# 236088/reflect-sampling-nerf

Measured on AMD Instinct MI355X. Metric: rays/sec (train step) at 4096 rays x 128 samples, 1/2/4/8 MI355X; PSNR vs ref, higher is better.
Workload: dtype f32

## Files before the change

### reflect_sampling_nerf_amd/csrc/rsn_field_bwd.hip

```cpp
#include "rsn_mfma.h"

#include "rsn_field_common.h"
#include "rsn_field_bwd_common.h"

template <int NB, int MMA>
__global__ __launch_bounds__(256) void rsn_field_bwd_kernel(const BwdJobs J) {
  constexpr bool FOLD = MMA == RSN_MMA_F32_FOLDED;
  constexpr int MODE = FOLD ? 0 : MMA;
  constexpr int HIT = FOLD ? 16 : NB * 4;
  constexpr int XITS = (NB * 4 > 16) ? NB * 4 : 16;
  constexpr int WAVE_F4 = (XITS + RSN_AUX_ITS) * 64;
  constexpr int W = NB * 32;
  constexpr bool SBF = MODE == 3;
  __shared__ float4 smem[4 * WAVE_F4];

  const int lane = threadIdx.x & 63;
  const int wid = __builtin_amdgcn_readfirstlane(threadIdx.x >> 6);
  float4* X = smem + wid * WAVE_F4 + lane;
  float* Xf = reinterpret_cast<float*>(X);

  const BwdShared& P = J.s;
  const TileJobs T = tile_space<128>(J);
  const float* __restrict__ pk = P.packed;
  const float4 zero4 = make_float4(0.0f, 0.0f, 0.0f, 0.0f);

  for (long long gtile = blockIdx.x; gtile < T.n_tiles; gtile += gridDim.x) {
    const TileAt ta = tile_at(T, gtile);
    const BwdJob& a = J.j[ta.job];
    const long long n_points = ta.n_points, tile = ta.tile;
    const long long p0 = tile * 128 + wid * 32;
    if (p0 >= n_points) continue;
    int ln = lane;
    asm volatile("" : "+v"(ln));
    const int m = ln & 31, h = ln >> 5;
    const long long p = p0 + m;
    const bool valid = p < n_points;
    const long long pc = valid ? p : n_points - 1;
    const int rows = (int)(n_points - p0 < 32 ? n_points - p0 : 32);
    constexpr bool LOOPST = MODE == 0;
    auto rb_epi = [&](float* base, long long elem, int row_elems) {
      return rowbuf<SBF>(LOOPST ? nullptr : base, elem, rows, row_elems, m, h);
    };
    auto rb_loop = [&](float* base, long long elem, int row_elems) {
      return rowbuf<false>(LOOPST ? base : nullptr, elem, rows, row_elems, m, h);
    };
    const float live = valid ? 1.0f : 0.0f;

    auto bits_at = [&](int l) -> const unsigned* {
      return a.saved.relu_bits + ((((long long)l * (a.act_stride / W)) + pc) * 2 + h) * (NB / 2 > 2 ? NB / 2 : 2);
    };
    HeadGradIn hg;
    head_grad_inputs(a, pc, live, h == 1 && valid, hg);

    X[0] = (h == 1) ? make_float4(hg.dz[0], hg.dz[1], hg.dz[2], 0.0f) : zero4;
    X[64] = zero4; X[128] = zero4; X[192] = zero4;
    {
      const ReluBits<4> mb = load_relu_bits<4>(bits_at(P.num_layers));
      __builtin_amdgcn_sched_barrier(0);
      f32x16 acc[4];
      zero_acc<4>(acc);
      gemm_mode<MODE, 4, 4, true>(acc, pk + P.L.wT_rgb, pk + P.L.hT_rgb, X, 4, ln);
      store_masked_bits<4, SBF>(acc, X, mb, h, rb_epi(a.gout.da_mid, p0 * 128, 128));
    }
    if constexpr (!FOLD) {
      f32x16 acc[NB];
      zero_acc<NB>(acc);
      gemm_mode<MODE, NB, NB, true>(acc, pk + P.L.wT_mid_x, pk + P.L.hT_mid_x, X, 16, ln, rb_loop(a.gout.da_mid, p0 * 128, 128));
      store_act<NB, NB, false, SBF>(acc, X, rb_epi(a.gout.d_bott, p0 * W, W), h);
    }
    {
      const float4 q0 = head_grad_row<false>(h == 0 ? 0 : 1, a, P.density_bias, pc, live, hg);
      const float4 q1 = head_grad_row<false>(h == 0 ? 2 : 3, a, P.density_bias, pc, live, hg);
      X[(HIT + 0) * 64] = q0;
      X[(HIT + 1) * 64] = q1;
      X[(HIT + 2) * 64] = zero4;
      X[(HIT + 3) * 64] = zero4;
      if (valid && a.gout.dz_heads) {
        *reinterpret_cast<float4*>(a.gout.dz_heads + pc * 16 + 4 * h) = q0;
        *reinterpret_cast<float4*>(a.gout.dz_heads + pc * 16 + 8 + 4 * h) = q1;
      }
      const int l = P.num_layers - 1;
      const ReluBits<NB> mb = load_relu_bits<NB>(bits_at(l));
      __builtin_amdgcn_sched_barrier(0);
      f32x16 acc[NB];
      zero_acc<NB>(acc);
      if constexpr (FOLD)
        gemm_mode<MODE, NB, NB, true>(acc, pk + P.L.wT_fold, pk + P.L.hT_bh, X, 16 + 4, ln, rb_loop(a.gout.da_mid, p0 * 128, 128));
      else
        gemm_mode<MODE, NB, NB, true>(acc, pk + P.L.wT_bh, pk + P.L.hT_bh, X, NB * 4 + 4, ln, rb_loop(a.gout.d_bott, p0 * W, W));
      store_masked_bits<NB, SBF>(acc, X, mb, h, rb_epi(a.gout.dy, (long long)l * a.act_stride + p0 * W, W));
    }
    f32x16 eacc[4];
    zero_acc<4>(eacc);
#pragma unroll 1
    for (int l = P.num_layers - 1; l >= 1; --l) {
      if (a.need_input_grad && l == P.skip_layer)
        gemm_mode<MODE, 4, 4, true>(eacc, pk + P.L.wT_enc_skip, pk + P.L.hT_enc_skip, X, NB * 4, ln);
      const ReluBits<NB> mb = load_relu_bits<NB>(bits_at(l - 1));
      __builtin_amdgcn_sched_barrier(0);
      f32x16 acc[NB];
      zero_acc<NB>(acc);
      gemm_mode<MODE, NB, NB, true>(acc, pk + P.L.wT_x[l], pk + P.L.hT_x[l], X, NB * 4, ln,
                          rb_loop(a.gout.dy, (long long)l * a.act_stride + p0 * W, W));
      store_masked_bits<NB, SBF>(acc, X, mb, h, rb_epi(a.gout.dy, (long long)(l - 1) * a.act_stride + p0 * W, W));
    }
    if (LOOPST && !a.need_input_grad) {
      const RowBuf r0 = rb_loop(a.gout.dy, p0 * W, W);
#pragma unroll 4
      for (int it = 0; it < NB * 4; ++it) sv_put_it(r0, it, X[it * 64]);
    }
    if (a.need_input_grad) {
      gemm_mode<MODE, 4, 4, true>(eacc, pk + P.L.wT_enc0, pk + P.L.hT_enc0, X, NB * 4, ln, rb_loop(a.gout.dy, p0 * W, W));
      store_act<4, 4, false>(eacc, X);
      const float* encp = a.saved.enc + pc * RSN_K_ENC_PAD;
      float dvar[3];
#pragma unroll 1
      for (int c = 0; c < 3; ++c) {
        float part = 0.0f;
#pragma unroll 2
        for (int jj = 0; jj < 8; ++jj) {
          const float f = h ? P.freqs[8 + jj] : P.freqs[jj];
          const int u = c * 8 + jj, u2 = u + 24;
          const float gs = Xf[(u >> 2) * 256 + (u & 3)], gc = Xf[(u2 >> 2) * 256 + (u2 & 3)];
          const float fs = encp[(u >> 2) * 8 + 4 * h + (u & 3)], fc = encp[(u2 >> 2) * 8 + 4 * h + (u2 & 3)];
          part += (-0.5f * (f * f)) * (gs * fs + gc * fc);
        }
        const float tot = part + __shfl_xor(part, 32, 64);
        if (c == 0) dvar[0] = tot; else if (c == 1) dvar[1] = tot; else dvar[2] = tot;
      }
      if (h == 0 && valid && a.gout.d_input) a.gout.d_input[pc] = input_grad_of_dvar(a, pc, dvar);
    }
  }
}

static int launch_bwd_jobs(const rsn_field_desc* d, const float* packed, BwdJob* js, int n, void* stream) {
  RSN_REQUIRE(n >= 1 && n <= RSN_MAX_JOBS, RSN_ERR_INVALID_ARGUMENT, "n_jobs=%d (1..%d)", n, RSN_MAX_JOBS);
  BwdJobs J = {};
  RSN_TRY(rsn_fill_shared(J.s, d, packed));
  for (int k = 0; k < n; ++k) {
    BwdJob& a = js[k];
    RSN_REQUIRE(a.saved.relu_bits && a.saved.heads && a.gout.dy, RSN_ERR_INVALID_ARGUMENT,
                "job %d: saved relu_bits / heads and gout.dy are required", k);
    RSN_REQUIRE(!a.need_input_grad || (a.saved.enc && a.gout.d_input), RSN_ERR_INVALID_ARGUMENT,
                "job %d: need_input_grad needs saved.enc and gout.d_input", k);
    RSN_REQUIRE(a.mode == RSN_MODE_INF || (a.fwd.raw_density && a.fwd.diff && a.fwd.tint), RSN_ERR_INVALID_ARGUMENT,
// ... 94 lines not shown
```

### reflect_sampling_nerf_amd/csrc/rsn_mfma.h

```cpp
#pragma once
#include "rsn_common.h"

typedef float f32x16 __attribute__((ext_vector_type(16)));

#define RSN_MODE_FRUSTUM 0
#define RSN_MODE_INF 1
#define RSN_MODE_GAUSS 2
#define RSN_MODE_EMB 3

__device__ __forceinline__ float softplus_f(float x) { return x > 20.0f ? x : log1pf(expf(x)); }
__device__ __forceinline__ float sigmoid_f(float x) { return 1.0f / (1.0f + expf(-x)); }

__device__ __forceinline__ float sincos_big(float a, int quad) {
  const float q = rintf(a * 0.63661977236758134308f);
  float r = __builtin_fmaf(-q, 1.5707963705062866f, a);
  r = __builtin_fmaf(-q, -4.371138828673793e-08f, r);
  r = __builtin_fmaf(-q, -1.7151245100058819e-15f, r);
  const int n = (int)q + quad;
  const float s = r * r;
  const float ps = r + r * s * (-1.6666654611e-1f + s * (8.3321608736e-3f + s * (-1.9515295891e-4f)));
  const float pc =
      1.0f + s * (-0.5f + s * (4.166664568298827e-2f + s * (-1.388731625493765e-3f + s * 2.443315711809948e-5f)));
  const float v = (n & 1) ? pc : ps;
  return (n & 2) ? -v : v;
// ... 176 lines not shown
  int it = 0;
#pragma unroll 1
  for (; it + 2 < n_it; it += 3) {
    load_w<NBO, NBT>(wc, wp, cl(it + 2));
    b1 = xl[cl(it + 1) * 64];
    mma4<NBO>(acc, wa, b0);
    if (sv_on(save)) sv_put_it(save, it, b0);
    interleave_loads<NBO>();
    __builtin_amdgcn_sched_barrier(0);
    load_w<NBO, NBT>(wa, wp, cl(it + 3));
    b2 = xl[cl(it + 2) * 64];
    mma4<NBO>(acc, wb, b1);
    if (sv_on(save)) sv_put_it(save, it + 1, b1);
    interleave_loads<NBO>();
    __builtin_amdgcn_sched_barrier(0);
    load_w<NBO, NBT>(wb, wp, cl(it + 4));
    b0 = xl[cl(it + 3) * 64];
    mma4<NBO>(acc, wc, b2);
    if (sv_on(save)) sv_put_it(save, it + 2, b2);
    interleave_loads<NBO>();
    __builtin_amdgcn_sched_barrier(0);
  }
  if (it < n_it) {
    mma4<NBO>(acc, wa, b0);
    if (sv_on(save)) sv_put_it(save, it, b0);
  }
  if (it + 1 < n_it) {
    b1 = xl[(it + 1) * 64];
    mma4<NBO>(acc, wb, b1);
    if (sv_on(save)) sv_put_it(save, it + 1, b1);
  }
}

template <int NBO, int NBT = NBO, class SV = const float*>
__device__ __forceinline__ void gemm_run(f32x16 (&acc)[NBO], float4 (&wa)[NBO], const float* __restrict__ wseg,
                                          const float4* xl, int n_it, int lane, SV save = nullptr) {
  const WBuf wp = wbuf_make(wseg, lane);
  float4 wb[NBO];
  float4 ba, bb;
  ba = xl[0];
  int it = 0;
#pragma unroll 1
  for (; it + 1 < n_it; it += 2) {
    load_w<NBO, NBT>(wb, wp, it + 1);
    bb = xl[(it + 1) * 64];
    mma4<NBO>(acc, wa, ba);
    if (sv_on(save)) sv_put_it(save, it, ba);
    interleave_loads<NBO>();
    __builtin_amdgcn_sched_barrier(0);
    {
      const int in = (it + 2 < n_it) ? it + 2 : n_it - 1;
      load_w<NBO, NBT>(wa, wp, in);
      ba = xl[in * 64];
    }
    mma4<NBO>(acc, wb, bb);
    if (sv_on(save)) sv_put_it(save, it + 1, bb);
    interleave_loads<NBO>();
    __builtin_amdgcn_sched_barrier(0);
  }
  if (it < n_it) {
    mma4<NBO>(acc, wa, ba);
    if (sv_on(save)) sv_put_it(save, it, ba);
  }
}

template <int NBO, int NBT = NBO, bool PF2 = false, class SV = const float*>
// ... 111 lines not shown
    xhi = xl[(2 * k2 + 1) * 64];
    __builtin_amdgcn_sched_barrier(0);
    if (H1 > 0) mma16<NBO, (H1 > 0 ? H1 : 1), (H1 > 0 ? H0 : 0), NSPLIT, FULL>(acc, wb, bc);
    __builtin_amdgcn_sched_barrier(0);
    bc = bn;
  }
}

template <int MODE, int NBO, int NBT = NBO, bool PF2 = false, class SV = const float*>
__device__ __forceinline__ void gemm_mode(f32x16 (&acc)[NBO], const float* __restrict__ w32, const float* __restrict__ w16,
                                          const float4* xl, int n_it, int lane, SV save = nullptr) {
  static_assert(MODE == 0 || NBT == NBO, "the split-bf16 loops own every output block of their segment");
  if (MODE == 0) {
    gemm<NBO, NBT, PF2>(acc, w32, xl, n_it, lane, save);
  } else {
    gemm_bf16<NBO, (MODE == 1 ? 3 : (MODE == 2 ? 2 : 1))>(acc, w16, xl, (n_it + 1) / 2, lane);
  }
}

template <int MODE, int NBO, int NBT = NBO>
__device__ __forceinline__ void pre_mode(float4 (&wa)[NBO], const float* __restrict__ w32, int lane) {
  if (MODE == 0) pre_w<NBO, NBT>(wa, w32, lane);
}

template <int MODE, int NBO, int NBT = NBO, bool PF2 = false, class SV = const float*>
__device__ __forceinline__ void gemm_mode_run(f32x16 (&acc)[NBO], float4 (&wa)[NBO], const float* __restrict__ w32,
                                              const float* __restrict__ w16, const float4* xl, int n_it, int lane,
                                              SV save = nullptr) {
  static_assert(MODE == 0 || NBT == NBO, "the split-bf16 loops own every output block of their segment");
  if (MODE == 0) {
    if (PF2) gemm_run2<NBO, NBT>(acc, wa, w32, xl, n_it, lane, save); else gemm_run<NBO, NBT>(acc, wa, w32, xl, n_it, lane, save);
  } else {
    gemm_bf16<NBO, (MODE == 1 ? 3 : (MODE == 2 ? 2 : 1))>(acc, w16, xl, (n_it + 1) / 2, lane);
  }
}

template <int NBO>
__device__ __forceinline__ void zero_acc(f32x16 (&acc)[NBO]) {
#pragma unroll
  for (int nb = 0; nb < NBO; ++nb)
#pragma unroll
    for (int r = 0; r < 16; ++r) acc[nb][r] = 0.0f;
}

__device__ __forceinline__ unsigned relu_bits16(const f32x16& a) {
  unsigned b = 0u;
#pragma unroll
  for (int r = 0; r < 16; ++r) {
    const unsigned lo = __float_as_uint(relu_f(a[r]));
    unsigned bit;
    if (r == 0) {
      asm("v_min_u32 %0, %1, 1" : "=v"(bit) : "v"(lo));
      b = bit;
    } else {
      unsigned nb;
      asm("v_min_u32 %0, %2, 1\n\tv_lshl_or_b32 %1, %0, %3, %4" : "=&v"(bit), "=v"(nb) : "v"(lo), "n"(r), "v"(b));
      b = nb;
    }
  }
  return b;
}

template <int Q>
__device__ __forceinline__ unsigned relu_bits4q(unsigned b, const float4 v) {
  const unsigned lo[4] = {__float_as_uint(v.x), __float_as_uint(v.y), __float_as_uint(v.z), __float_as_uint(v.w)};
#pragma unroll
// ... 153 lines not shown
    c = __builtin_amdgcn_mfma_f32_32x32x16_bf16(s3, b, c, 0, 0, 0);
    c = __builtin_amdgcn_mfma_f32_32x32x16_bf16(s2, b, c, 0, 0, 0);
    c = __builtin_amdgcn_mfma_f32_32x32x16_bf16(s1, b, c, 0, 0, 0);
    acc[nb0 + t] = c;
  }
}

template <int NBO>
__device__ __forceinline__ void gemm_f32_bits(f32x16 (&acc)[NBO], const float* __restrict__ w32seg, const float* __restrict__ wd,
                                              const ReluBits<NBO>& m, int lane) {
  static_assert(NBO % 2 == 0, "two fragment buffers of NBO / 2 blocks");
  constexpr int NH = NBO / 2, NK = 2 * NBO;
  const WBuf wp = wbuf_make(w32seg, lane);
  const float* __restrict__ wdl = wd + 4 * (lane >> 5);
  float4 fa[NH][2], fb[NH][2];
  load_w32_pair<NBO, NH>(fa, wp, 0, 0);
  const SeedWords mw = seed_words<NBO>(m);
  float4 dlo = *reinterpret_cast<const float4*>(wdl), dhi = *reinterpret_cast<const float4*>(wdl + 8);
#pragma unroll 1
  for (int kk = 0; kk < NK; ++kk) {
    load_w32_pair<NBO, NH>(fb, wp, kk, NH);
    const int kn = (kk + 1 < NK) ? kk + 1 : kk;
    const float4 nlo = *reinterpret_cast<const float4*>(wdl + 16 * kn), nhi = *reinterpret_cast<const float4*>(wdl + 16 * kn + 8);
    const bf16x8 bc = bits_bf16x8(mw, kk);
    mma16_bits_f32<NBO, NH>(acc, fa, dlo, dhi, bc, 0);
    __builtin_amdgcn_sched_barrier(0);
    load_w32_pair<NBO, NH>(fa, wp, kn, 0);
    mma16_bits_f32<NBO, NH>(acc, fb, dlo, dhi, bc, NH);
    __builtin_amdgcn_sched_barrier(0);
    dlo = nlo; dhi = nhi;
  }
}

__device__ __forceinline__ f32x16 x9_block(f32x16 c, const BSplit& w, const BSplit& b) {
  c = __builtin_amdgcn_mfma_f32_32x32x16_bf16(w.s3, b.s3, c, 0, 0, 0);
  c = __builtin_amdgcn_mfma_f32_32x32x16_bf16(w.s3, b.s2, c, 0, 0, 0);
  c = __builtin_amdgcn_mfma_f32_32x32x16_bf16(w.s2, b.s3, c, 0, 0, 0);
  c = __builtin_amdgcn_mfma_f32_32x32x16_bf16(w.s3, b.s1, c, 0, 0, 0);
  c = __builtin_amdgcn_mfma_f32_32x32x16_bf16(w.s2, b.s2, c, 0, 0, 0);
  c = __builtin_amdgcn_mfma_f32_32x32x16_bf16(w.s1, b.s3, c, 0, 0, 0);
  c = __builtin_amdgcn_mfma_f32_32x32x16_bf16(w.s2, b.s1, c, 0, 0, 0);
  c = __builtin_amdgcn_mfma_f32_32x32x16_bf16(w.s1, b.s2, c, 0, 0, 0);
  c = __builtin_amdgcn_mfma_f32_32x32x16_bf16(w.s1, b.s1, c, 0, 0, 0);
  return c;
}

template <int NBO>
__device__ __forceinline__ void gemm_f32_x9(f32x16 (&acc)[NBO], const float* __restrict__ w32seg, const float4* xl, int n_k16,
                                            int lane) {
  static_assert(NBO % 2 == 0, "two fragment buffers of NBO / 2 blocks");
  constexpr int NH = NBO / 2;
  const WBuf wp = wbuf_make(w32seg, lane);
  float4 fa[NH][2], fb[NH][2];
  load_w32_pair<NBO, NH>(fa, wp, 0, 0);
  load_w32_pair<NBO, NH>(fb, wp, 0, NH);
  BSplit bc = split8<3>(xl[0], xl[64]);
  const int k1 = n_k16 > 1 ? 1 : 0;
  float4 xlo = xl[(2 * k1) * 64], xhi = xl[(2 * k1 + 1) * 64];
  BSplit w = split8<3>(fa[0][0], fa[0][1]);
  BSplit bn = bc;
#pragma unroll 1
  for (int kk = 0; kk < n_k16; ++kk) {
    const int kn = (kk + 1 < n_k16) ? kk + 1 : kk;
    const int k2 = (kk + 2 < n_k16) ? kk + 2 : kn;
#pragma unroll
    for (int b = 0; b < NBO; ++b) {
      BSplit wn;
      if (b + 1 < NH) wn = split8<3>(fa[b + 1][0], fa[b + 1][1]);
      else if (b + 1 < NBO) wn = split8<3>(fb[b + 1 - NH][0], fb[b + 1 - NH][1]);
      else wn = split8<3>(fa[0][0], fa[0][1]);
      if (b == NH - 1) load_w32_pair<NBO, NH>(fa, wp, kn, 0);
      if (b == NBO - 1) {
        load_w32_pair<NBO, NH>(fb, wp, kn, NH);
        bn = split8<3>(xlo, xhi);
        xlo = xl[(2 * k2) * 64];
        xhi = xl[(2 * k2 + 1) * 64];
      }
      acc[b] = x9_block(acc[b], w, bc);
      const bool loads = b == NH - 1 || b == NBO - 1;
#pragma unroll
      for (int g = 0; g < 9; ++g) {
        __builtin_amdgcn_sched_group_barrier(0x008, 1, 0);
        if (loads && g < 2 * NH) __builtin_amdgcn_sched_group_barrier(0x020, 1, 0);
        if (b == NBO - 1) __builtin_amdgcn_sched_group_barrier(0x002, 8, 0);
        else __builtin_amdgcn_sched_group_barrier(0x002, 5, 0);
      }
      if (b == NBO - 1) __builtin_amdgcn_sched_group_barrier(0x100, 2, 0);
      __builtin_amdgcn_sched_barrier(0);
      w = wn;
    }
    bc = bn;
  }
}

__device__ __forceinline__ unsigned bit_mask(int word, int pos) {
  unsigned m;
  asm("v_bfe_i32 %0, %1, %2, 1" : "=v"(m) : "v"(word), "n"(pos));
  return m;
}

template <int NBO, bool SBF = false, class SV = float*>
__device__ __forceinline__ void store_masked_bits(const f32x16 (&acc)[NBO], float4* xl, const ReluBits<NBO>& m, int h,
                                                  SV save = nullptr) {
#pragma unroll
  for (int nb = 0; nb < NBO; ++nb)
#pragma unroll
    for (int q = 0; q < 4; ++q) {
      const int word = m.w[nb / 2];
      const int base = (nb & 1) * 16 + 4 * q;
      float4 v;
      v.x = __uint_as_float(__float_as_uint(acc[nb][4 * q + 0]) & bit_mask(word, base + 0));
      v.y = __uint_as_float(__float_as_uint(acc[nb][4 * q + 1]) & bit_mask(word, base + 1));
      v.z = __uint_as_float(__float_as_uint(acc[nb][4 * q + 2]) & bit_mask(word, base + 2));
      v.w = __uint_as_float(__float_as_uint(acc[nb][4 * q + 3]) & bit_mask(word, base + 3));
      xl[(nb * 4 + q) * 64] = v;
      if (sv_on(save)) sv_put<SBF>(save, nb, q, h, v);
    }
}

template <int NBO, int NBS, bool RELU, bool SBF = false, class SV = float*>
__device__ __forceinline__ void store_act(const f32x16 (&acc)[NBO], float4* xl, SV save = nullptr, int h = 0,
                                          unsigned* bits = nullptr) {
  unsigned bw[NBS / 2 > 0 ? NBS / 2 : 1];
#pragma unroll
  for (int nb = 0; nb < NBS; ++nb) {
    unsigned b16 = 0u;
#pragma unroll
    for (int q = 0; q < 4; ++q) {
      float4 v = make_float4(acc[nb][4 * q + 0], acc[nb][4 * q + 1], acc[nb][4 * q + 2], acc[nb][4 * q + 3]);
      if (RELU) {
        v.x = relu_f(v.x);
        v.y = relu_f(v.y);
        v.z = relu_f(v.z);
        v.w = relu_f(v.w);
        b16 = relu_bits4(b16, v, q);
      }
      xl[(nb * 4 + q) * 64] = v;
      if (sv_on(save)) sv_put<SBF>(save, nb, q, h, v);
    }
    if (RELU) {
      if (nb & 1) bw[nb / 2] |= b16 << 16; else bw[nb / 2] = b16;
    }
  }
  if (RELU && bits) {
    if (NBS >= 8) {
#pragma unroll
      for (int w4 = 0; w4 < NBS / 8; ++w4)
        *reinterpret_cast<uint4*>(bits + w4 * 4) = make_uint4(bw[w4 * 4], bw[w4 * 4 + 1], bw[w4 * 4 + 2], bw[w4 * 4 + 3]);
    } else {
// ... 92 lines not shown
```

### reflect_sampling_nerf_amd/csrc/rsn_field_kernel.h

```cpp
#pragma once
#include "rsn_mfma.h"

#include "rsn_field_common.h"

template <bool X9, bool PACKED, int MODE, int NBO>
__device__ __forceinline__ void sweep_gemm(f32x16 (&acc)[NBO], const float* __restrict__ w32, const float* __restrict__ w16,
                                           const float4* xl, int n_it, int lane) {
  if constexpr (X9) {
    if constexpr (PACKED) gemm_bf16<NBO, 3, true>(acc, w16, xl, n_it / 2, lane); else gemm_f32_x9<NBO>(acc, w32, xl, n_it / 2, lane);
  } else {
    gemm_mode<MODE, NBO, NBO, true>(acc, w32, w16, xl, n_it, lane);
  }
}

template <int NB, bool TRAIN, int MMA>
__global__ __launch_bounds__(256) void rsn_field_kernel(const FieldJobs J) {
  constexpr bool FOLD = MMA == RSN_MMA_F32_FOLDED;
  constexpr int MODE = FOLD ? 0 : MMA;
  static_assert(!FOLD || TRAIN, "the folded bottleneck serves the exact-fp32 training kernels");
  constexpr int NBH = FOLD ? 5 : NB + 1;
  constexpr int XITS = (NB * 4 > 16) ? NB * 4 : 16;
  constexpr int WAVE_F4 = (XITS + RSN_AUX_ITS) * 64;
  constexpr int W = NB * 32;
  constexpr bool SBF = TRAIN && MODE == 3;
  __shared__ float4 smem[4 * WAVE_F4];

  const int lane = threadIdx.x & 63;
  const int wid = __builtin_amdgcn_readfirstlane(threadIdx.x >> 6);
  float4* X = smem + wid * WAVE_F4 + lane;
  float4* AUX = X + XITS * 64;
  float* Xf = reinterpret_cast<float*>(X);

  const FieldShared& P = J.s;
  const TileJobs T = tile_space<128>(J);
  const float* __restrict__ pk = P.packed;

  for (long long gtile = blockIdx.x; gtile < T.n_tiles; gtile += gridDim.x) {
    const TileAt ta = tile_at(T, gtile);
    const FieldJob& a = J.j[ta.job];
    const long long n_points = ta.n_points, tile = ta.tile;
    const long long p0 = tile * 128 + wid * 32;
    if (p0 >= n_points) continue;
    int ln = lane;
    asm volatile("" : "+v"(ln));
    const int m = ln & 31, h = ln >> 5;
// ... 190 lines not shown
      if (h == 1 && valid) colour_out<false, TRAIN>(a, pc, accr[0][0], accr[0][1], accr[0][2], dcol, tcol);
    }

    constexpr bool SEED_BITS = TRAIN && MODE == 0;
    if (TRAIN && a.saved.normals && a.saved.relu_bits) {
      const float* __restrict__ wd = pk + P.L.v_density;
      const bool peel = SEED_BITS && P.num_layers >= 2;
      if (peel) {
        const ReluBits<NB> m7 = load_relu_bits<NB>(bits_at(P.num_layers - 1));
        const ReluBits<NB> mb = load_relu_bits<NB>(bits_at(P.num_layers - 2));
        __builtin_amdgcn_sched_barrier(0);
        f32x16 acc[NB];
        zero_acc<NB>(acc);
        if constexpr (FOLD) {
          gemm_bf16_bits<NB>(acc, pk + P.L.hT_seed, m7, ln);
        } else {
          gemm_f32_bits<NB>(acc, pk + P.L.wT_x[P.num_layers - 1], wd, m7, ln);
        }
        store_masked_bits<NB>(acc, X, mb, h);
      } else {
        const ReluBits<NB> mb = load_relu_bits<NB>(bits_at(P.num_layers - 1));
#pragma unroll
        for (int it = 0; it < NB * 4; ++it) {
          const float4 w = *reinterpret_cast<const float4*>(wd + it * 8 + 4 * h);
          const int word = mb.w[it / 8];
          const int base = ((it / 4) & 1) * 16 + 4 * (it & 3);
          X[it * 64] = make_float4(
              __uint_as_float(__float_as_uint(w.x) & bit_mask(word, base + 0)),
              __uint_as_float(__float_as_uint(w.y) & bit_mask(word, base + 1)),
              __uint_as_float(__float_as_uint(w.z) & bit_mask(word, base + 2)),
              __uint_as_float(__float_as_uint(w.w) & bit_mask(word, base + 3)));
        }
      }
      f32x16 eacc[4];
      zero_acc<4>(eacc);
#pragma unroll 1
      for (int l = P.num_layers - (peel ? 2 : 1); l >= 1; --l) {
        if (l == P.skip_layer) sweep_gemm<SEED_BITS, FOLD, MODE, 4>(eacc, pk + P.L.wT_enc_skip, pk + P.L.hT_enc_skip, X, NB * 4, ln);
        const ReluBits<NB> mb = load_relu_bits<NB>(bits_at(l - 1));
        __builtin_amdgcn_sched_barrier(0);
        f32x16 acc[NB];
        zero_acc<NB>(acc);
        sweep_gemm<SEED_BITS, FOLD, MODE, NB>(acc, pk + P.L.wT_x[l], pk + P.L.hT_x[l], X, NB * 4, ln);
        store_masked_bits<NB>(acc, X, mb, h);
      }
      sweep_gemm<SEED_BITS, FOLD, MODE, 4>(eacc, pk + P.L.wT_enc0, pk + P.L.hT_enc0, X, NB * 4, ln);
      store_act<4, 4, false>(eacc, X);
      float nrm[3];
#pragma unroll 1
      for (int c = 0; c < 3; ++c) {
        const float x = (c == 0) ? mc[0] : (c == 1 ? mc[1] : mc[2]);
        const float v = (c == 0) ? vc[0] : (c == 1 ? vc[1] : vc[2]);
        const float sx = 6.283185307179586f * x;
        float part = 0.0f;
#pragma unroll 2
        for (int jj = 0; jj < 8; ++jj) {
          const float f = h ? P.freqs[8 + jj] : P.freqs[jj];
          const float ang = sx * f;
          const float e = has_cov ? expf(-0.5f * (v * (f * f))) : 1.0f;
          const int u = c * 8 + jj;
          const float gs = Xf[(u >> 2) * 256 + (u & 3)];
          const float gc = Xf[((u + 24) >> 2) * 256 + ((u + 24) & 3)];
          part += (gs * (e * cos_big(ang)) + gc * (e * cos_big(ang + 1.5707963267948966f))) * f;
        }
        part *= 6.283185307179586f;
        if (h == 0) part += Xf[12 * 256 + c];
        const float tot = part + __shfl_xor(part, 32, 64);
        if (c == 0) nrm[0] = tot; else if (c == 1) nrm[1] = tot; else nrm[2] = tot;
      }
      if (h == 0 && valid) {
        const float len = fmaxf(sqrtf(nrm[0] * nrm[0] + nrm[1] * nrm[1] + nrm[2] * nrm[2]), 1e-12f);
        a.saved.normals[pc * 3 + 0] = -(nrm[0] / len);
        a.saved.normals[pc * 3 + 1] = -(nrm[1] / len);
        a.saved.normals[pc * 3 + 2] = -(nrm[2] / len);
      }
    }
  }
}
```

Measured before the change: 94550.

## Chain weight prefetch across successive backward GEMM segments

Replaces each per-layer GEMM call in the backward field kernel with a chained variant. During the tail iterations of one segment it loads the first one or two weight fragments of the next segment, so every GEMM after the first starts with its weights already in registers. This targets the global-load latency bubble at each layer boundary. The cost is more live registers (fa/fb/sa/sb are kept across the tile loop) and fragile fragment bookkeeping across the FOLD, NB and need_input_grad paths, which could hurt occupancy or correctness.

```diff
diff --git a/reflect_sampling_nerf_amd/csrc/rsn_field_bwd.hip b/reflect_sampling_nerf_amd/csrc/rsn_field_bwd.hip
--- a/reflect_sampling_nerf_amd/csrc/rsn_field_bwd.hip
+++ b/reflect_sampling_nerf_amd/csrc/rsn_field_bwd.hip
@@ -23,6 +23,14 @@
   const TileJobs T = tile_space<128>(J);
   const float* __restrict__ pk = P.packed;
   const float4 zero4 = make_float4(0.0f, 0.0f, 0.0f, 0.0f);
+
+  float4 fa[NB], fb[NB], sa[4], sb[4];
+  if constexpr (MODE == 0) {
+    const WBuf wp = wbuf_make(pk + P.L.wT_rgb, lane);
+    load_w<4>(sa, wp, 0);
+    load_w<4>(sb, wp, 1);
+  }
+  constexpr const float* no_rows = nullptr;
 
   for (long long gtile = blockIdx.x; gtile < T.n_tiles; gtile += gridDim.x) {
     const TileAt ta = tile_at(T, gtile);
@@ -49,6 +57,9 @@
     auto bits_at = [&](int l) -> const unsigned* {
       return a.saved.relu_bits + ((((long long)l * (a.act_stride / W)) + pc) * 2 + h) * (NB / 2 > 2 ? NB / 2 : 2);
     };
+    auto seg_behind = [&](int l) -> const float* {
+      return pk + (l > 1 ? P.L.wT_x[l - 1] : (a.need_input_grad ? P.L.wT_enc0 : P.L.wT_rgb));
+    };
     HeadGradIn hg;
     head_grad_inputs(a, pc, live, h == 1 && valid, hg);
 
@@ -59,13 +70,15 @@
       __builtin_amdgcn_sched_barrier(0);
       f32x16 acc[4];
       zero_acc<4>(acc);
-      gemm_mode<MODE, 4, 4, true>(acc, pk + P.L.wT_rgb, pk + P.L.hT_rgb, X, 4, ln);
+      gemm_mode_chain<MODE, 4, 4, NB>(acc, sa, sb, pk + P.L.wT_rgb, pk + P.L.hT_rgb, X, ln, no_rows,
+                                      pk + (FOLD ? P.L.wT_fold : P.L.wT_mid_x), fa, fb);
       store_masked_bits<4, SBF>(acc, X, mb, h, rb_epi(a.gout.da_mid, p0 * 128, 128));
     }
     if constexpr (!FOLD) {
       f32x16 acc[NB];
       zero_acc<NB>(acc);
-      gemm_mode<MODE, NB, NB, true>(acc, pk + P.L.wT_mid_x, pk + P.L.hT_mid_x, X, 16, ln, rb_loop(a.gout.da_mid, p0 * 128, 128));
+      gemm_mode_chain<MODE, 16, NB, NB>(acc, fa, fb, pk + P.L.wT_mid_x, pk + P.L.hT_mid_x, X, ln, rb_loop(a.gout.da_mid, p0 * 128, 128),
+                                        pk + P.L.wT_bh, fa, fb);
       store_act<NB, NB, false, SBF>(acc, X, rb_epi(a.gout.d_bott, p0 * W, W), h);
     }
     {
@@ -85,9 +98,11 @@
       f32x16 acc[NB];
       zero_acc<NB>(acc);
       if constexpr (FOLD)
-        gemm_mode<MODE, NB, NB, true>(acc, pk + P.L.wT_fold, pk + P.L.hT_bh, X, 16 + 4, ln, rb_loop(a.gout.da_mid, p0 * 128, 128));
+        gemm_mode_chain<MODE, 16 + 4, NB, NB>(acc, fa, fb, pk + P.L.wT_fold, pk + P.L.hT_bh, X, ln, rb_loop(a.gout.da_mid, p0 * 128, 128),
+                                              seg_behind(P.num_layers), fa, fb);
       else
-        gemm_mode<MODE, NB, NB, true>(acc, pk + P.L.wT_bh, pk + P.L.hT_bh, X, NB * 4 + 4, ln, rb_loop(a.gout.d_bott, p0 * W, W));
+        gemm_mode_chain<MODE, NB * 4 + 4, NB, NB>(acc, fa, fb, pk + P.L.wT_bh, pk + P.L.hT_bh, X, ln, rb_loop(a.gout.d_bott, p0 * W, W),
+                                                  seg_behind(P.num_layers), fa, fb);
       store_masked_bits<NB, SBF>(acc, X, mb, h, rb_epi(a.gout.dy, (long long)l * a.act_stride + p0 * W, W));
     }
     f32x16 eacc[4];
@@ -100,17 +115,19 @@
       __builtin_amdgcn_sched_barrier(0);
       f32x16 acc[NB];
       zero_acc<NB>(acc);
-      gemm_mode<MODE, NB, NB, true>(acc, pk + P.L.wT_x[l], pk + P.L.hT_x[l], X, NB * 4, ln,
-                          rb_loop(a.gout.dy, (long long)l * a.act_stride + p0 * W, W));
+      gemm_mode_chain<MODE, NB * 4, NB, NB>(acc, fa, fb, pk + P.L.wT_x[l], pk + P.L.hT_x[l], X, ln,
+                          rb_loop(a.gout.dy, (long long)l * a.act_stride + p0 * W, W), seg_behind(l), fa, fb);
       store_masked_bits<NB, SBF>(acc, X, mb, h, rb_epi(a.gout.dy, (long long)(l - 1) * a.act_stride + p0 * W, W));
     }
+    if constexpr (MODE == 0) chain_head4<NB>(sa, sb, fa, fb, seg_behind(1), ln);
     if (LOOPST && !a.need_input_grad) {
       const RowBuf r0 = rb_loop(a.gout.dy, p0 * W, W);
 #pragma unroll 4
       for (int it = 0; it < NB * 4; ++it) sv_put_it(r0, it, X[it * 64]);
     }
     if (a.need_input_grad) {
-      gemm_mode<MODE, 4, 4, true>(eacc, pk + P.L.wT_enc0, pk + P.L.hT_enc0, X, NB * 4, ln, rb_loop(a.gout.dy, p0 * W, W));
+      gemm_mode_chain<MODE, NB * 4, 4, 4>(eacc, sa, sb, pk + P.L.wT_enc0, pk + P.L.hT_enc0, X, ln, rb_loop(a.gout.dy, p0 * W, W),
+                                          pk + P.L.wT_rgb, sa, sb);
       store_act<4, 4, false>(eacc, X);
       const float* encp = a.saved.enc + pc * RSN_K_ENC_PAD;
       float dvar[3];
diff --git a/reflect_sampling_nerf_amd/csrc/rsn_mfma.h b/reflect_sampling_nerf_amd/csrc/rsn_mfma.h
--- a/reflect_sampling_nerf_amd/csrc/rsn_mfma.h
+++ b/reflect_sampling_nerf_amd/csrc/rsn_mfma.h
@@ -232,6 +232,77 @@
   }
 }
 
+template <int NL, bool LDS>
+__device__ __forceinline__ void interleave_loads_n() {
+#pragma unroll
+  for (int g = 0; g < NL; ++g) {
+    __builtin_amdgcn_sched_group_barrier(0x008, 1, 0);
+    __builtin_amdgcn_sched_group_barrier(0x020, 1, 0);
+  }
+  if (LDS) {
+    __builtin_amdgcn_sched_group_barrier(0x008, 1, 0);
+    __builtin_amdgcn_sched_group_barrier(0x100, 1, 0);
+  }
+}
+
+template <int N_IT, int NBO, int NBN, int DEPTH = 2, class SV = const float*>
+__device__ __forceinline__ void gemm_run2_chain(f32x16 (&acc)[NBO], const float4 (&w0)[NBO], const float4 (&w1)[NBO],
+                                                 const float* __restrict__ wseg, const float4* xl, int lane, SV save,
+                                                 const float* __restrict__ nseg, float4 (&n0)[NBN], float4 (&n1)[NBN]) {
+  static_assert(N_IT >= 3 && (DEPTH == 1 || DEPTH == 2), "a tail of three to five K-iterations; one or two fragments ahead");
+  constexpr int R = 3 + N_IT % 3, N_LOOP = N_IT - R;
+  const WBuf wp = wbuf_make(wseg, lane), np = wbuf_make(nseg, lane);
+  float4 wa[NBO], wb[NBO], wc[NBO];
+  float4 b0, b1, b2;
+#pragma unroll
+  for (int nb = 0; nb < NBO; ++nb) wa[nb] = w0[nb];
+  if constexpr (DEPTH == 2) {
+#pragma unroll
+    for (int nb = 0; nb < NBO; ++nb) wb[nb] = w1[nb];
+  } else {
+    load_w<NBO>(wb, wp, 1);
+  }
+  b0 = xl[0];
+#pragma unroll 1
+  for (int it = 0; it < N_LOOP; it += 3) {
+    load_w<NBO>(wc, wp, it + 2);
+    b1 = xl[(it + 1) * 64];
+    mma4<NBO>(acc, wa, b0);
+    if (sv_on(save)) sv_put_it(save, it, b0);
+    interleave_loads<NBO>();
+    __builtin_amdgcn_sched_barrier(0);
+    load_w<NBO>(wa, wp, it + 3);
+    b2 = xl[(it + 2) * 64];
+    mma4<NBO>(acc, wb, b1);
+    if (sv_on(save)) sv_put_it(save, it + 1, b1);
+    interleave_loads<NBO>();
+    __builtin_amdgcn_sched_barrier(0);
+    load_w<NBO>(wb, wp, it + 4);
+    b0 = xl[(it + 3) * 64];
+    mma4<NBO>(acc, wc, b2);
+    if (sv_on(save)) sv_put_it(save, it + 2, b2);
+    interleave_loads<NBO>();
+    __builtin_amdgcn_sched_barrier(0);
+  }
+  auto step = [&](auto jc, const float4 (&wcur)[NBO], const float4 bcur, float4 (&wld)[NBO], float4& bnx) {
+    constexpr int j = decltype(jc)::value, i = N_LOOP + j;
+    constexpr bool own = j + 2 < R, nx = !own && (j + 2 == R || DEPTH == 2);
+    if constexpr (own) load_w<NBO>(wld, wp, i + 2);
+    else if constexpr (j + 2 == R) load_w<NBN>(n0, np, 0);
+    else if constexpr (DEPTH == 2) load_w<NBN>(n1, np, 1);
+    if constexpr (j + 1 < R) bnx = xl[(i + 1) * 64];
+    mma4<NBO>(acc, wcur, bcur);
+    if (sv_on(save)) sv_put_it(save, i, bcur);
+    interleave_loads_n<(own ? NBO : (nx ? NBN : 0)), (j + 1 < R)>();
+    __builtin_amdgcn_sched_barrier(0);
+  };
+  step(std::integral_constant<int, 0>(), wa, b0, wc, b1);
+  step(std::integral_constant<int, 1>(), wb, b1, wa, b2);
+  step(std::integral_constant<int, 2>(), wc, b2, wb, b0);
+  if constexpr (R > 3) step(std::integral_constant<int, 3>(), wa, b0, wc, b1);
+  if constexpr (R > 4) step(std::integral_constant<int, 4>(), wb, b1, wa, b2);
+}
+
 template <int NBO, int NBT = NBO, class SV = const float*>
 __device__ __forceinline__ void gemm_run(f32x16 (&acc)[NBO], float4 (&wa)[NBO], const float* __restrict__ wseg,
                                           const float4* xl, int n_it, int lane, SV save = nullptr) {
@@ -409,6 +480,31 @@
     if (PF2) gemm_run2<NBO, NBT>(acc, wa, w32, xl, n_it, lane, save); else gemm_run<NBO, NBT>(acc, wa, w32, xl, n_it, lane, save);
   } else {
     gemm_bf16<NBO, (MODE == 1 ? 3 : (MODE == 2 ? 2 : 1))>(acc, w16, xl, (n_it + 1) / 2, lane);
+  }
+}
+
+template <int MODE, int N_IT, int NBO, int NBN, class SV = const float*>
+__device__ __forceinline__ void gemm_mode_chain(f32x16 (&acc)[NBO], const float4 (&w0)[NBO], const float4 (&w1)[NBO],
+                                                const float* __restrict__ w32, const float* __restrict__ w16, const float4* xl,
+                                                int lane, SV save, const float* __restrict__ n32, float4 (&n0)[NBN],
+                                                float4 (&n1)[NBN]) {
+  if constexpr (MODE == 0) gemm_run2_chain<N_IT, NBO, NBN>(acc, w0, w1, w32, xl, lane, save, n32, n0, n1);
+  else gemm_bf16<NBO, (MODE == 1 ? 3 : (MODE == 2 ? 2 : 1))>(acc, w16, xl, (N_IT + 1) / 2, lane);
+}
+
+template <int NB>
+__device__ __forceinline__ void chain_head4(float4 (&w0)[4], float4 (&w1)[4], const float4 (&n0)[NB], const float4 (&n1)[NB],
+                                            const float* __restrict__ seg, int lane) {
+  static_assert(NB == 2 || NB == 4 || NB == 8, "widths 64, 128, 256");
+  if constexpr (NB == 8) {
+#pragma unroll
+    for (int nb = 0; nb < 4; ++nb) { w0[nb] = n0[nb]; w1[nb] = n0[4 + nb]; }
+  } else if constexpr (NB == 4) {
+#pragma unroll
+    for (int nb = 0; nb < 4; ++nb) { w0[nb] = n0[nb]; w1[nb] = n1[nb]; }
+  } else {
+    w0[0] = n0[0]; w0[1] = n0[1]; w0[2] = n1[0]; w0[3] = n1[1];
+    load_w<4>(w1, wbuf_make(seg, lane), 1);
   }
 }
 
```

New measurement: 94760 (median of 3 runs). No clear change (+0.2%).

## Switch seed-bits backward sweep to 16x16x32 MFMA tiles with new layout

Applied to the files above, without the earlier changes.

Replaces the 32x32x16 bf16 MFMA x9-split GEMM used in the seed-bits backward trunk sweep with a 16x16x32 variant, for both the folded packed-bf16 and fp32 x9 paths. It adds new weight load helpers, a lane mapping for 16-wide tiles, per-half relu-bit loading, and masked stores matching the new accumulator layout. The aim is better MFMA throughput or latency hiding and a larger K per instruction. The cost is a new fragment/LDS layout that must line up with how weights are packed, and possible extra register pressure.

```diff
diff --git a/reflect_sampling_nerf_amd/csrc/rsn_field_kernel.h b/reflect_sampling_nerf_amd/csrc/rsn_field_kernel.h
--- a/reflect_sampling_nerf_amd/csrc/rsn_field_kernel.h
+++ b/reflect_sampling_nerf_amd/csrc/rsn_field_kernel.h
@@ -3,14 +3,16 @@
 
 #include "rsn_field_common.h"
 
-template <bool X9, bool PACKED, int MODE, int NBO>
+template <int MODE, int NBO>
 __device__ __forceinline__ void sweep_gemm(f32x16 (&acc)[NBO], const float* __restrict__ w32, const float* __restrict__ w16,
                                            const float4* xl, int n_it, int lane) {
-  if constexpr (X9) {
-    if constexpr (PACKED) gemm_bf16<NBO, 3, true>(acc, w16, xl, n_it / 2, lane); else gemm_f32_x9<NBO>(acc, w32, xl, n_it / 2, lane);
-  } else {
-    gemm_mode<MODE, NBO, NBO, true>(acc, w32, w16, xl, n_it, lane);
-  }
+  gemm_mode<MODE, NBO, NBO, true>(acc, w32, w16, xl, n_it, lane);
+}
+template <bool PACKED, int N_IT, int NBO>
+__device__ __forceinline__ void sweep_gemm(f32x4 (&acc)[NBO][2][2], const float* __restrict__ w32, const float* __restrict__ w16,
+                                           const float4* xl, int lane) {
+  static_assert(N_IT % 4 == 0, "K = 8 N_IT is a multiple of 32 at every width (the units are padded to 32): no tail path");
+  if constexpr (PACKED) gemm_bf16_s16<NBO>(acc, w16, xl, N_IT / 4, lane); else gemm_f32_x9_s16<NBO>(acc, w32, xl, N_IT / 4, lane);
 }
 
 template <int NB, bool TRAIN, int MMA>
@@ -267,20 +269,41 @@
               __uint_as_float(__float_as_uint(w.w) & bit_mask(word, base + 3)));
         }
       }
-      f32x16 eacc[4];
-      zero_acc<4>(eacc);
-#pragma unroll 1
-      for (int l = P.num_layers - (peel ? 2 : 1); l >= 1; --l) {
-        if (l == P.skip_layer) sweep_gemm<SEED_BITS, FOLD, MODE, 4>(eacc, pk + P.L.wT_enc_skip, pk + P.L.hT_enc_skip, X, NB * 4, ln);
-        const ReluBits<NB> mb = load_relu_bits<NB>(bits_at(l - 1));
-        __builtin_amdgcn_sched_barrier(0);
-        f32x16 acc[NB];
-        zero_acc<NB>(acc);
-        sweep_gemm<SEED_BITS, FOLD, MODE, NB>(acc, pk + P.L.wT_x[l], pk + P.L.hT_x[l], X, NB * 4, ln);
-        store_masked_bits<NB>(acc, X, mb, h);
-      }
-      sweep_gemm<SEED_BITS, FOLD, MODE, 4>(eacc, pk + P.L.wT_enc0, pk + P.L.hT_enc0, X, NB * 4, ln);
-      store_act<4, 4, false>(eacc, X);
+      if constexpr (SEED_BITS) {
+        auto bits16_at = [&](int l, int ph) -> const unsigned* {
+          const long long q = p0 + (ln & 15) + 16 * ph, qc = q < n_points ? q : n_points - 1;
+          return a.saved.relu_bits + ((((long long)l * (a.act_stride / W)) + qc) * 2 + ((ln >> 4) & 1)) * (NB / 2 > 2 ? NB / 2 : 2);
+        };
+        f32x4 eacc[4][2][2];
+        zero_acc16<4>(eacc);
+#pragma unroll 1
+        for (int l = P.num_layers - (peel ? 2 : 1); l >= 1; --l) {
+          if (l == P.skip_layer) sweep_gemm<FOLD, NB * 4, 4>(eacc, pk + P.L.wT_enc_skip, pk + P.L.hT_enc_skip, X, ln);
+          const ReluBits<NB> mb[2] = {load_relu_bits<NB>(bits16_at(l - 1, 0)), load_relu_bits<NB>(bits16_at(l - 1, 1))};
+          __builtin_amdgcn_sched_barrier(0);
+          f32x4 acc[NB][2][2];
+          zero_acc16<NB>(acc);
+          sweep_gemm<FOLD, NB * 4, NB>(acc, pk + P.L.wT_x[l], pk + P.L.hT_x[l], X, ln);
+          store_masked_bits16<NB>(acc, X, mb, ln);
+        }
+        sweep_gemm<FOLD, NB * 4, 4>(eacc, pk + P.L.wT_enc0, pk + P.L.hT_enc0, X, ln);
+        store_act16<4>(eacc, X, ln);
+      } else {
+        f32x16 eacc[4];
+        zero_acc<4>(eacc);
+#pragma unroll 1
+        for (int l = P.num_layers - 1; l >= 1; --l) {
+          if (l == P.skip_layer) sweep_gemm<MODE, 4>(eacc, pk + P.L.wT_enc_skip, pk + P.L.hT_enc_skip, X, NB * 4, ln);
+          const ReluBits<NB> mb = load_relu_bits<NB>(bits_at(l - 1));
+          __builtin_amdgcn_sched_barrier(0);
+          f32x16 acc[NB];
+          zero_acc<NB>(acc);
+          sweep_gemm<MODE, NB>(acc, pk + P.L.wT_x[l], pk + P.L.hT_x[l], X, NB * 4, ln);
+          store_masked_bits<NB>(acc, X, mb, h);
+        }
+        sweep_gemm<MODE, 4>(eacc, pk + P.L.wT_enc0, pk + P.L.hT_enc0, X, NB * 4, ln);
+        store_act<4, 4, false>(eacc, X);
+      }
       float nrm[3];
 #pragma unroll 1
       for (int c = 0; c < 3; ++c) {
diff --git a/reflect_sampling_nerf_amd/csrc/rsn_mfma.h b/reflect_sampling_nerf_amd/csrc/rsn_mfma.h
--- a/reflect_sampling_nerf_amd/csrc/rsn_mfma.h
+++ b/reflect_sampling_nerf_amd/csrc/rsn_mfma.h
@@ -628,64 +628,168 @@
   }
 }
 
-__device__ __forceinline__ f32x16 x9_block(f32x16 c, const BSplit& w, const BSplit& b) {
-  c = __builtin_amdgcn_mfma_f32_32x32x16_bf16(w.s3, b.s3, c, 0, 0, 0);
-  c = __builtin_amdgcn_mfma_f32_32x32x16_bf16(w.s3, b.s2, c, 0, 0, 0);
-  c = __builtin_amdgcn_mfma_f32_32x32x16_bf16(w.s2, b.s3, c, 0, 0, 0);
-  c = __builtin_amdgcn_mfma_f32_32x32x16_bf16(w.s3, b.s1, c, 0, 0, 0);
-  c = __builtin_amdgcn_mfma_f32_32x32x16_bf16(w.s2, b.s2, c, 0, 0, 0);
-  c = __builtin_amdgcn_mfma_f32_32x32x16_bf16(w.s1, b.s3, c, 0, 0, 0);
-  c = __builtin_amdgcn_mfma_f32_32x32x16_bf16(w.s2, b.s1, c, 0, 0, 0);
-  c = __builtin_amdgcn_mfma_f32_32x32x16_bf16(w.s1, b.s2, c, 0, 0, 0);
-  c = __builtin_amdgcn_mfma_f32_32x32x16_bf16(w.s1, b.s1, c, 0, 0, 0);
-  return c;
-}
-
-template <int NBO>
-__device__ __forceinline__ void gemm_f32_x9(f32x16 (&acc)[NBO], const float* __restrict__ w32seg, const float4* xl, int n_k16,
-                                            int lane) {
-  static_assert(NBO % 2 == 0, "two fragment buffers of NBO / 2 blocks");
-  constexpr int NH = NBO / 2;
-  const WBuf wp = wbuf_make(w32seg, lane);
-  float4 fa[NH][2], fb[NH][2];
-  load_w32_pair<NBO, NH>(fa, wp, 0, 0);
-  load_w32_pair<NBO, NH>(fb, wp, 0, NH);
-  BSplit bc = split8<3>(xl[0], xl[64]);
-  const int k1 = n_k16 > 1 ? 1 : 0;
-  float4 xlo = xl[(2 * k1) * 64], xhi = xl[(2 * k1 + 1) * 64];
-  BSplit w = split8<3>(fa[0][0], fa[0][1]);
-  BSplit bn = bc;
+typedef float f32x4 __attribute__((ext_vector_type(4)));
+
+template <int NBO>
+__device__ __forceinline__ void zero_acc16(f32x4 (&acc)[NBO][2][2]) {
+#pragma unroll
+  for (int nb = 0; nb < NBO; ++nb)
+#pragma unroll
+    for (int q = 0; q < 4; ++q) acc[nb][q >> 1][q & 1] = f32x4{0.0f, 0.0f, 0.0f, 0.0f};
+}
+
+struct Lane16 {
+  int ol;
+  int kh;
+};
+__device__ __forceinline__ Lane16 lane16(int lane) {
+  Lane16 g;
+  g.ol = (lane & 15) + 2 * (lane & 16);
+  g.kh = lane >> 5;
+  return g;
+}
+
+__device__ __forceinline__ bf16x8 piece(const BSplit& b, int k) { return k == 0 ? b.s1 : (k == 1 ? b.s2 : b.s3); }
+constexpr int x9_wp(int p) { constexpr int t[9] = {2, 2, 1, 2, 1, 0, 1, 0, 0}; return t[p]; }
+constexpr int x9_bp(int p) { constexpr int t[9] = {2, 1, 2, 0, 1, 2, 0, 1, 0}; return t[p]; }
+template <int NBO, int NQ>
+__device__ __forceinline__ void mma16s(f32x4 (&acc)[NBO][2][2], const bf16x8 (&w)[NQ][2][3], const BSplit (&b)[2], int nb0) {
+#pragma unroll
+  for (int t = 0; t < NQ; ++t)
+#pragma unroll
+    for (int p = 0; p < 9; ++p)
+#pragma unroll
+      for (int q = 0; q < 4; ++q)
+        acc[nb0 + t][q >> 1][q & 1] = __builtin_amdgcn_mfma_f32_16x16x32_bf16(w[t][q >> 1][x9_wp(p)], piece(b[q & 1], x9_bp(p)),
+                                                                              acc[nb0 + t][q >> 1][q & 1], 0, 0, 0);
+}
+
+template <int NQ>
+__device__ __forceinline__ void load_w16s(bf16x8 (&w)[NQ][2][3], const WBuf& wp, int s, int nbo, int nb0) {
+#pragma unroll
+  for (int t = 0; t < NQ; ++t)
+#pragma unroll
+    for (int rh = 0; rh < 2; ++rh)
+#pragma unroll
+      for (int sp = 0; sp < 3; ++sp) {
+        const u32x4 v = __builtin_amdgcn_raw_buffer_load_b128(wp.r, wp.voff + rh * 256u, (unsigned)(((2 * s * nbo + nb0 + t) * 3 + sp) * 1024), 0);
+        w[t][rh][sp] = __builtin_bit_cast(bf16x8, v);
+      }
+}
+
+template <int NBO>
+__device__ __forceinline__ void gemm_bf16_s16(f32x4 (&acc)[NBO][2][2], const float* __restrict__ wseg, const float4* xl, int n_k32,
+                                              int lane) {
+  static_assert(NBO % 2 == 0, "an even number of fragment buffers' worth of blocks");
+  constexpr int NQ = NBO >= 4 ? NBO / 4 : 1, NC = NBO / NQ;
+  const Lane16 g = lane16(lane);
+  WBuf wp = wbuf_make(wseg, lane);
+  wp.voff = (unsigned)g.ol * 16u + (unsigned)g.kh * (NBO * 3072u);
+  const float4* xb = xl - lane + g.ol + g.kh * 128;
+  bf16x8 wa[NQ][2][3], wb[NQ][2][3];
+  load_w16s<NQ>(wa, wp, 0, NBO, 0);
+  BSplit bc[2] = {split8<3>(xb[0], xb[64]), split8<3>(xb[16], xb[80])};
+  const int s1 = n_k32 > 1 ? 1 : 0;
+  float4 x0lo = xb[4 * s1 * 64], x0hi = xb[(4 * s1 + 1) * 64], x1lo = xb[4 * s1 * 64 + 16], x1hi = xb[(4 * s1 + 1) * 64 + 16];
 #pragma unroll 1
-  for (int kk = 0; kk < n_k16; ++kk) {
-    const int kn = (kk + 1 < n_k16) ? kk + 1 : kk;
-    const int k2 = (kk + 2 < n_k16) ? kk + 2 : kn;
-#pragma unroll
-    for (int b = 0; b < NBO; ++b) {
-      BSplit wn;
-      if (b + 1 < NH) wn = split8<3>(fa[b + 1][0], fa[b + 1][1]);
-      else if (b + 1 < NBO) wn = split8<3>(fb[b + 1 - NH][0], fb[b + 1 - NH][1]);
-      else wn = split8<3>(fa[0][0], fa[0][1]);
-      if (b == NH - 1) load_w32_pair<NBO, NH>(fa, wp, kn, 0);
-      if (b == NBO - 1) {
-        load_w32_pair<NBO, NH>(fb, wp, kn, NH);
-        bn = split8<3>(xlo, xhi);
-        xlo = xl[(2 * k2) * 64];
-        xhi = xl[(2 * k2 + 1) * 64];
+  for (int s = 0; s < n_k32; ++s) {
+    const int sn = (s + 1 < n_k32) ? s + 1 : s;
+    const int s2 = (s + 2 < n_k32) ? s + 2 : sn;
+    BSplit bn[2];
+#pragma unroll
+    for (int c = 0; c < NC; ++c) {
+      if (c & 1) load_w16s<NQ>(wa, wp, c + 1 < NC ? s : sn, NBO, c + 1 < NC ? (c + 1) * NQ : 0);
+      else load_w16s<NQ>(wb, wp, s, NBO, (c + 1) * NQ);
+      __builtin_amdgcn_sched_barrier(0);
+      if (c == 0) bn[0] = split8<3>(x0lo, x0hi);
+      if (c == 1) bn[1] = split8<3>(x1lo, x1hi);
+      if (c == NC - 1) {
+        x0lo = xb[4 * s2 * 64]; x0hi = xb[(4 * s2 + 1) * 64];
+        x1lo = xb[4 * s2 * 64 + 16]; x1hi = xb[(4 * s2 + 1) * 64 + 16];
       }
-      acc[b] = x9_block(acc[b], w, bc);
-      const bool loads = b == NH - 1 || b == NBO - 1;
-#pragma unroll
-      for (int g = 0; g < 9; ++g) {
+      if (c & 1) mma16s<NBO, NQ>(acc, wb, bc, c * NQ); else mma16s<NBO, NQ>(acc, wa, bc, c * NQ);
+#pragma unroll
+      for (int m = 0; m < NQ * 36; ++m) {
         __builtin_amdgcn_sched_group_barrier(0x008, 1, 0);
-        if (loads && g < 2 * NH) __builtin_amdgcn_sched_group_barrier(0x020, 1, 0);
-        if (b == NBO - 1) __builtin_amdgcn_sched_group_barrier(0x002, 8, 0);
-        else __builtin_amdgcn_sched_group_barrier(0x002, 5, 0);
+        if (c < 2) __builtin_amdgcn_sched_group_barrier(0x002, 2, 0);
       }
-      if (b == NBO - 1) __builtin_amdgcn_sched_group_barrier(0x100, 2, 0);
+      if (c == NC - 1) __builtin_amdgcn_sched_group_barrier(0x100, 4, 0);
+      __builtin_amdgcn_sched_barrier(0);
+    }
+    bc[0] = bn[0];
+    bc[1] = bn[1];
+  }
+}
+
+template <int NQ>
+__device__ __forceinline__ void load_w32s(float4 (&f)[NQ][2][2], const WBuf& b, int s, int nbo, int nb0) {
+#pragma unroll
+  for (int t = 0; t < NQ; ++t)
+#pragma unroll
+    for (int rh = 0; rh < 2; ++rh)
+#pragma unroll
+      for (int j = 0; j < 2; ++j) {
+        const u32x4 v = __builtin_amdgcn_raw_buffer_load_b128(b.r, b.voff + rh * 256u, (unsigned)(((4 * s + j) * nbo + nb0 + t) * 1024), 0);
+        f[t][rh][j] = make_float4(__uint_as_float(v.x), __uint_as_float(v.y), __uint_as_float(v.z), __uint_as_float(v.w));
+      }
+}
+
+template <int NBO>
+__device__ __forceinline__ void gemm_f32_x9_s16(f32x4 (&acc)[NBO][2][2], const float* __restrict__ w32seg, const float4* xl,
+                                                int n_k32, int lane) {
+  static_assert(NBO % 2 == 0, "an even number of fragment buffers' worth of blocks");
+  constexpr int NQ = NBO >= 4 ? NBO / 4 : 1, NC = NBO / NQ, UQ = 2 * NQ, NU = 2 * NBO;
+  const Lane16 g = lane16(lane);
+  WBuf wp = wbuf_make(w32seg, lane);
+  wp.voff = (unsigned)g.ol * 16u + (unsigned)g.kh * (NBO * 2048u);
+  const float4* xb = xl - lane + g.ol + g.kh * 128;
+  float4 fa[NQ][2][2], fb[NQ][2][2];
+  load_w32s<NQ>(fa, wp, 0, NBO, 0);
+  load_w32s<NQ>(fb, wp, 0, NBO, NQ);
+  BSplit bc[2] = {split8<3>(xb[0], xb[64]), split8<3>(xb[16], xb[80])};
+  const int s1 = n_k32 > 1 ? 1 : 0;
+  float4 x0lo = xb[4 * s1 * 64], x0hi = xb[(4 * s1 + 1) * 64], x1lo = xb[4 * s1 * 64 + 16], x1hi = xb[(4 * s1 + 1) * 64 + 16];
+  BSplit w = split8<3>(fa[0][0][0], fa[0][0][1]);
+  BSplit bn[2] = {bc[0], bc[1]};
+#pragma unroll 1
+  for (int s = 0; s < n_k32; ++s) {
+    const int sn = (s + 1 < n_k32) ? s + 1 : s;
+    const int s2 = (s + 2 < n_k32) ? s + 2 : sn;
+#pragma unroll
+    for (int u = 0; u < NU; ++u) {
+      const int un = (u + 1) % NU, cn = (un / UQ) & 1, tn = (un / 2) % NQ;
+      const BSplit wn = cn ? split8<3>(fb[tn][un & 1][0], fb[tn][un & 1][1]) : split8<3>(fa[tn][un & 1][0], fa[tn][un & 1][1]);
+      const bool reload = u % UQ == UQ - 1;
+      if (reload) {
+        const int c = u / UQ, c2 = (c + 2) % NC;
+        if (c & 1) load_w32s<NQ>(fb, wp, c + 2 < NC ? s : sn, NBO, c2 * NQ);
+        else load_w32s<NQ>(fa, wp, c + 2 < NC ? s : sn, NBO, c2 * NQ);
+      }
+      if (u == NU - 2) bn[0] = split8<3>(x0lo, x0hi);
+      if (u == NU - 1) {
+        bn[1] = split8<3>(x1lo, x1hi);
+        x0lo = xb[4 * s2 * 64]; x0hi = xb[(4 * s2 + 1) * 64];
+        x1lo = xb[4 * s2 * 64 + 16]; x1hi = xb[(4 * s2 + 1) * 64 + 16];
+      }
+#pragma unroll
+      for (int p = 0; p < 9; ++p)
+#pragma unroll
+        for (int ph = 0; ph < 2; ++ph)
+          acc[u >> 1][u & 1][ph] = __builtin_amdgcn_mfma_f32_16x16x32_bf16(piece(w, x9_wp(p)), piece(bc[ph], x9_bp(p)),
+                                                                           acc[u >> 1][u & 1][ph], 0, 0, 0);
+#pragma unroll
+      for (int m = 0; m < 18; ++m) {
+        __builtin_amdgcn_sched_group_barrier(0x008, 1, 0);
+        if (reload && m < NQ * 4) __builtin_amdgcn_sched_group_barrier(0x020, 1, 0);
+        if (u >= NU - 2) __builtin_amdgcn_sched_group_barrier(0x002, 6, 0);
+        else __builtin_amdgcn_sched_group_barrier(0x002, 3, 0);
+      }
+      if (u == NU - 1) __builtin_amdgcn_sched_group_barrier(0x100, 4, 0);
       __builtin_amdgcn_sched_barrier(0);
       w = wn;
     }
-    bc = bn;
+    bc[0] = bn[0];
+    bc[1] = bn[1];
   }
 }
 
@@ -711,6 +815,42 @@
       v.w = __uint_as_float(__float_as_uint(acc[nb][4 * q + 3]) & bit_mask(word, base + 3));
       xl[(nb * 4 + q) * 64] = v;
       if (sv_on(save)) sv_put<SBF>(save, nb, q, h, v);
+    }
+}
+
+template <int NBO>
+__device__ __forceinline__ void store_masked_bits16(const f32x4 (&acc)[NBO][2][2], float4* xl, const ReluBits<NBO> (&m)[2], int lane) {
+  const Lane16 g = lane16(lane);
+  float4* xs = xl - lane + g.ol + g.kh * 64;
+#pragma unroll
+  for (int ph = 0; ph < 2; ++ph)
+#pragma unroll
+    for (int nb = 0; nb < NBO; ++nb) {
+      const int word = (int)(m[ph].w[nb / 2] >> (4 * g.kh));
+#pragma unroll
+      for (int rh = 0; rh < 2; ++rh) {
+        const int base = (nb & 1) * 16 + 8 * rh;
+        const f32x4& a = acc[nb][rh][ph];
+        float4 v;
+        v.x = __uint_as_float(__float_as_uint(a[0]) & bit_mask(word, base + 0));
+        v.y = __uint_as_float(__float_as_uint(a[1]) & bit_mask(word, base + 1));
+        v.z = __uint_as_float(__float_as_uint(a[2]) & bit_mask(word, base + 2));
+        v.w = __uint_as_float(__float_as_uint(a[3]) & bit_mask(word, base + 3));
+        xs[(nb * 4 + 2 * rh) * 64 + 16 * ph] = v;
+      }
+    }
+}
+
+template <int NBO>
+__device__ __forceinline__ void store_act16(const f32x4 (&acc)[NBO][2][2], float4* xl, int lane) {
+  const Lane16 g = lane16(lane);
+  float4* xs = xl - lane + g.ol + g.kh * 64;
+#pragma unroll
+  for (int nb = 0; nb < NBO; ++nb)
+#pragma unroll
+    for (int q = 0; q < 4; ++q) {
+      const f32x4& a = acc[nb][q >> 1][q & 1];
+      xs[(nb * 4 + 2 * (q >> 1)) * 64 + 16 * (q & 1)] = make_float4(a[0], a[1], a[2], a[3]);
     }
 }
 
```

Result: faster. 93960 before, 95350 after (median of 6 runs) (+1.5%).
